# YukunXia/SuperPoint-Stereo-Visual-Odometry

Measured on AMD Instinct MI355X. Metric: stereo frames/sec (1241x376 KITTI), higher is better.
Workload: dtype f32

## Files before the change

### superpoint-stereo-visual-odometry_amd/csrc/conv_wino4.hip.h

```cpp
#pragma once
#include <hip/hip_runtime.h>
#include <stdint.h>
#include <type_traits>
#include <vector>
#include "conv_mfma.hip.h"

#ifndef WINO4_LEAD
#define WINO4_LEAD 6
#endif
#ifndef WINO4_PRIO
#define WINO4_PRIO 1
#endif
#ifndef WINO4_H1_STEPS
#define WINO4_H1_STEPS 6
#endif
#ifndef WINO4_H1_START
#define WINO4_H1_START 3
#endif
#ifndef WINO4_H1_STRIDE
#define WINO4_H1_STRIDE 5
#endif
#ifndef WINO4_H2_START
#define WINO4_H2_START 4
#endif
#ifndef WINO4_H2_STRIDE
#define WINO4_H2_STRIDE 8
#endif
#ifndef WINO4_ABL
#define WINO4_ABL 0
#endif

#ifndef SPVO_STATIC_BANDS
#define SPVO_STATIC_BANDS 1
#endif

namespace spvo {

template <int TB>
struct Wino4TileT {
  static constexpr int CK = 4, TH = 8 * TB, TW = 32, LW = TW + 8, LH = TH + 2, NT = 16 * TB, NTH = 256 * TB;
  static constexpr int IN_FLOATS = CK * LH * LW;
  static constexpr int U_FLOATS = 36 * CK * CO_TILE;
  static constexpr int V_FLOATS = 10 * TB * 64 * 4;
  static constexpr int RAW_OFF = 0, U_OFF = 2 * IN_FLOATS, V_OFF = U_OFF + 2 * U_FLOATS;
  static constexpr int LDS_BYTES = (V_OFF + 2 * V_FLOATS) * 4 + 16;
};
using Wino4Tile = Wino4TileT<2>;

inline std::vector<float> pack_conv_weights_wino4(const float *w, const float *bias, int cout, int cin) {
  constexpr int CK = Wino4Tile::CK;
  const int co_tiles = (cout + CO_TILE - 1) / CO_TILE, nch = cin / CK;
  std::vector<float> out((size_t)co_tiles * nch * Wino4Tile::U_FLOATS + (size_t)co_tiles * CO_TILE, 0.f);
  static const double G[6][3] = {{0.25, 0, 0}, {-1.0 / 6, -1.0 / 6, -1.0 / 6}, {-1.0 / 6, 1.0 / 6, -1.0 / 6},
                                 {1.0 / 24, 1.0 / 12, 1.0 / 6}, {1.0 / 24, -1.0 / 12, 1.0 / 6}, {0, 0, 1}};
  for (int ct = 0; ct < co_tiles; ++ct)
    for (int o = 0; o < CO_TILE; ++o) {
      const int co = ct * CO_TILE + o;
      if (co >= cout) continue;
      out[(size_t)co_tiles * nch * Wino4Tile::U_FLOATS + co] = bias[co];
// ... 11 lines not shown
          }
      }
    }
  return out;
}

__device__ __forceinline__ void wino4_in6(const float x0, const float x1, const float x2, const float x3, const float x4, const float x5, float (&o)[6]) {
  const float e = fmaf(-4.f, x2, x4), od = fmaf(-4.f, x1, x3), e2 = x4 - x2, o2 = x3 - x1;
  o[0] = fmaf(4.f, x0, fmaf(-5.f, x2, x4));
  o[1] = e + od;
  o[2] = e - od;
  o[3] = fmaf(2.f, o2, e2);
  o[4] = fmaf(-2.f, o2, e2);
  o[5] = fmaf(4.f, x1, fmaf(-5.f, x3, x5));
}
__device__ __forceinline__ void wino4_out4(const float m0, const float m1, const float m2, const float m3, const float m4, const float m5, float (&y)[4]) {
  const float a = m1 + m2, b = m1 - m2, c = m3 + m4, d = m3 - m4;
  y[0] = (m0 + a) + c;
  y[1] = fmaf(2.f, d, b);
  y[2] = fmaf(4.f, c, a);
  y[3] = fmaf(8.f, d, b) + m5;
}

typedef float wino4_f32x2 __attribute__((ext_vector_type(2)));
__device__ __forceinline__ void wino4_out4(const wino4_f32x2 m0, const wino4_f32x2 m1, const wino4_f32x2 m2, const wino4_f32x2 m3, const wino4_f32x2 m4,
                                           const wino4_f32x2 m5, wino4_f32x2 (&y)[4]) {
  const wino4_f32x2 a = m1 + m2, b = m1 - m2, c = m3 + m4, d = m3 - m4;
  y[0] = (m0 + a) + c;
  y[1] = __builtin_elementwise_fma(wino4_f32x2{2.f, 2.f}, d, b);
  y[2] = __builtin_elementwise_fma(wino4_f32x2{4.f, 4.f}, c, a);
  y[3] = __builtin_elementwise_fma(wino4_f32x2{8.f, 8.f}, d, b) + m5;
}

template <bool POOL, bool RELU, int TAG = 0, int TB = 2>
__global__ __launch_bounds__(256 * TB, TB) void conv_wino4_kernel(const ConvArgs a) {
  using T = Wino4TileT<TB>;
  constexpr int CK = T::CK, LW = T::LW, LH = T::LH, LW4 = LW / 4, NTH = T::NTH;
  constexpr int IN_V4 = T::IN_FLOATS / 4;
  constexpr int U_V4 = T::U_FLOATS / 4;
  constexpr int NIT_U = (U_V4 + NTH - 1) / NTH;
  typedef float f32x2 __attribute__((ext_vector_type(2)));
  typedef float f32x4v __attribute__((ext_vector_type(4)));

  extern __shared__ __attribute__((aligned(16))) float smem[];

  const int tid = threadIdx.x;
  const int lane = tid & 63;
  const int c16 = lane & 15, g4 = lane >> 4;
  const int wave = __builtin_amdgcn_readfirstlane(tid >> 6);
  const int cq = wave & 3, tb = wave >> 2;
  const size_t in_plane = (size_t)a.in_hp * a.in_wp;
  const size_t out_plane = (size_t)a.out_hp * a.out_wp;
  const int n_tiles = a.tiles_x * a.tiles_y * a.co_tiles * a.batch;

  struct TileRef { const float *in_base, *w_base; int x0, y0, ct, img; };
  auto decode = [&](int id) {
    TileRef t;
    const int tx = id % a.tiles_x;
    id /= a.tiles_x;
    const int ty = id % a.tiles_y;
    id /= a.tiles_y;
    t.ct = id % a.co_tiles;
    t.img = id / a.co_tiles;
    t.x0 = tx * T::TW;
    t.y0 = ty * T::TH;
    t.in_base = a.in + ((size_t)t.img * a.in_ctot + a.in_coff) * in_plane + (size_t)(t.y0 + PADY - 1) * a.in_wp + (t.x0 + PADX - 4);
    t.w_base = a.wpack + (size_t)t.ct * a.n_chunks * T::U_FLOATS;
    return t;
  };

  auto raw_piece_off = [&](int idx) {
    idx = min(idx, IN_V4 - 1);
    const int ci = idx / (LH * LW4);
    const int rem = idx - ci * (LH * LW4);
    const int r = rem / LW4;
    const int q = rem - r * LW4;
    return 4u * (unsigned)(ci * (int)in_plane + r * a.in_wp + q * 4);
  };
  constexpr int R0 = NTH - 256;
  const unsigned roff0 = raw_piece_off(tid), roff1 = raw_piece_off(NTH + (tid - R0));
  const bool raw2 = tid >= R0 && NTH + (tid - R0) < IN_V4;
  auto issue_raw = [&](const TileRef &t, int chunk, float *buf) {
    const char *inb = reinterpret_cast<const char *>(t.in_base + (size_t)chunk * CK * in_plane);
    glds16(reinterpret_cast<const float *>(inb + roff0), buf + (wave * 64) * 4);
    if (raw2) glds16(reinterpret_cast<const float *>(inb + roff1), buf + (NTH + (wave - R0 / 64) * 64) * 4);
  };
  const unsigned uoff = 16u * (unsigned)tid;
  auto issue_u = [&](const TileRef &t, int chunk, float *buf) {
    const char *wb = reinterpret_cast<const char *>(t.w_base + (size_t)chunk * T::U_FLOATS);
#pragma unroll
    for (int it = 0; it < NIT_U; ++it)
      if (it < NIT_U - 1 || tid < U_V4 - (NIT_U - 1) * NTH) glds16(reinterpret_cast<const float *>(wb + (uoff + 16u * NTH * it)), buf + (it * NTH + wave * 64) * 4);
  };

  const int x_ci = TB == 2 ? (wave & 3) : 2 * (wave & 1) + ((lane >> 4) & 1), x_tile = TB == 2 ? (lane & 31) : (lane & 15), x_h = lane >> 5;
  const int x_trow = x_tile >> 3, x_tcol = x_tile & 7;
  const int raw_off = x_ci * (LH * LW) + (4 * x_trow + 3 * x_h) * LW + 4 * x_tcol + 3;
  const int v_off = x_h * (1280 * TB) + (x_tile >> 4) * 256 + (16 * x_ci + (x_tile & 15)) * 4;
  float xr[3][6];
  f32x4v xa[3];
  float xs0[3], xs1[3];
  auto xf_step = [&](const float *raw, float *vb, int st) {
    if (st < 3) {
      const float *d = raw + raw_off + st * LW;
      xs0[st] = d[0];
      xa[st] = *reinterpret_cast<const f32x4v *>(d + 1);
      xs1[st] = d[5];
    } else if (st < 6) {
      const int r = st - 3;
      wino4_in6(xs0[r], xa[r][0], xa[r][1], xa[r][2], xa[r][3], xs1[r], xr[r]);
    } else if (st == 6) {
#pragma unroll
      for (int r = 0; r < 3; ++r)
#pragma unroll
        for (int c = 0; c < 3; ++c) {
          typedef unsigned u32x2s __attribute__((ext_vector_type(2)));
          const u32x2s sw = __builtin_amdgcn_permlane32_swap(__float_as_uint(xr[r][c]), __float_as_uint(xr[r][c + 3]), false, false);
          xr[r][c] = __uint_as_float(sw[0]);
          xr[r][c + 3] = __uint_as_float(sw[1]);
        }
    } else {
      const int c = st - 7;
      float o[6];
      wino4_in6(xr[0][c], xr[1][c], xr[2][c], xr[0][c + 3], xr[1][c + 3], xr[2][c + 3], o);
#pragma unroll
      for (int i = 0; i < 6; ++i) vb[v_off + ((3 * i + c) >> 2) * (256 * TB) + ((3 * i + c) & 3)] = o[i];
    }
  };

  const int a_lane = cq * 64 + lane;
  const int b_lane = tb * 64 + lane;

  const int band = blockIdx.x & 7;
  auto wgs_before = [&](int b) { return min(b, (int)gridDim.x & 7) + b * ((int)gridDim.x >> 3); };
// ... 49 lines not shown
  Cursor cr = cu;
  advance(cr);
  asm volatile("s_waitcnt vmcnt(0)\n\ts_barrier" ::: "memory");
  if (wave < 2 * TB) {
#pragma unroll
    for (int st = 0; st < 10; ++st) xf_step(smem + T::RAW_OFF, smem + T::V_OFF, st);
  } else {
#pragma unroll
    for (int st = 0; st < WINO4_H1_STEPS; ++st) xf_step(smem + T::RAW_OFF + T::IN_FLOATS, smem + T::V_OFF + T::V_FLOATS, st);
  }
  asm volatile("s_waitcnt lgkmcnt(0)\n\ts_barrier" ::: "memory");
  if (cr.id < n_tiles) issue_raw(cr.t, cr.chunk, smem + T::RAW_OFF);
  advance(cr);

#ifdef WINO_STAMPS
  unsigned long long st_dma = 0, st_bar = 0, st_mfma = 0, st_epi = 0, st_items = 0, st_post = 0, st_bar_xf = 0, st_mfma_xf = 0;
  const unsigned long long st_t0 = __builtin_amdgcn_s_memtime(), st_r0 = __builtin_amdgcn_s_memrealtime();
  int st_c = 0;
#endif
  int k = 0;
  bool drained = false;
  constexpr unsigned OOB = 0xFFFFFFFFu;

  while (tile_id < n_tiles) {
    if (a.sched) {
      if (tid == 0) dyn_fetch = band_lo(band) + band_wgs(band) + atomicAdd(a.sched + band, 1);
    } else {
      nxt_id = tile_id + gridDim.x;
    }

    f32x4v acc[36];
    auto item = [&](auto first_tag, bool publish) {
      constexpr bool FIRST = decltype(first_tag)::value;
      const bool XF = __builtin_amdgcn_readfirstlane((wave >> TB) == (k & 1) ? 1 : 0) != 0;
#ifdef WINO_STAMPS
      const unsigned long long ts0 = __builtin_amdgcn_s_memtime();
#endif
      if (!drained) asm volatile("s_waitcnt vmcnt(0)" ::: "memory");
      drained = false;
#ifdef WINO_STAMPS
      const unsigned long long ts1 = __builtin_amdgcn_s_memtime();
#endif
      if (publish && tid == 0) *sched_slot = dyn_fetch < band_hi(band) ? dyn_fetch : n_tiles;
      asm volatile("s_waitcnt lgkmcnt(0)\n\ts_barrier" ::: "memory");
      if (publish) nxt_id = __builtin_amdgcn_readfirstlane(*sched_slot);
#ifdef WINO_STAMPS
      const unsigned long long ts2 = __builtin_amdgcn_s_memtime();
      st_dma += ts1 - ts0; st_bar += ts2 - ts1;
      if (st_c == 1) st_post += ts1 - ts0;
      if (XF) st_bar_xf += ts2 - ts1;
#endif
      const float *ub = smem + T::U_OFF + (k & 1) * T::U_FLOATS;
      const float *vb = smem + T::V_OFF + (k & 1) * T::V_FLOATS;
      float *u_next = smem + T::U_OFF + ((k + 1) & 1) * T::U_FLOATS;
      const float *raw_next2 = smem + T::RAW_OFF + (k & 1) * T::IN_FLOATS;
      float *raw_next3 = smem + T::RAW_OFF + ((k + 1) & 1) * T::IN_FLOATS;
      float *v_next = smem + T::V_OFF + ((k + 1) & 1) * T::V_FLOATS;
      const f32x4v *ub4 = reinterpret_cast<const f32x4v *>(ub) + a_lane;
      const f32x4v *vb4 = reinterpret_cast<const f32x4v *>(vb) + b_lane;
      constexpr int LEAD = WINO4_LEAD;
      f32x4v av[9], bv[10];
      auto b_piece = [](int p) { return 5 * (p / 18) + ((p % 18) >> 2); };
#pragma unroll
      for (int p = 0; p < ((WINO4_ABL & 8) ? 36 : LEAD); ++p) {
        if ((WINO4_ABL & 8) && k > 0) break;
        if ((p & 3) == 0) av[p >> 2] = ub4[(p >> 2) * 256];
        if (p == 0 || b_piece(p) != b_piece(p - 1)) bv[b_piece(p)] = vb4[b_piece(p) * (64 * TB)];
      }
#pragma unroll
      for (int p = 0; p < 36; ++p) {
        const int ph = p / 18, pq = p % 18, pos = 6 * (pq / 3) + 3 * ph + pq % 3;
        const float a_op = av[p >> 2][p & 3], b_op = bv[b_piece(p)][pq & 3];
#if WINO4_PRIO
#if WINO4_PRIO == 1
        if (p == 0) asm volatile("s_setprio 3");
        if (p == 9) asm volatile("s_setprio 2");
        if (p == 18) asm volatile("s_setprio 1");
        if (p == 27) asm volatile("s_setprio 0");
#elif WINO4_PRIO == 2
        if (p == 0) asm volatile("s_setprio 3");
        if (tb == 0) { if (p == 6) asm volatile("s_setprio 2"); if (p == 15) asm volatile("s_setprio 1"); if (p == 24) asm volatile("s_setprio 0"); }
        else { if (p == 12) asm volatile("s_setprio 2"); if (p == 24) asm volatile("s_setprio 1"); }
#elif WINO4_PRIO == 3
        if (p == 0) asm volatile("s_setprio 1");
        if (p == 18) asm volatile("s_setprio 0");
#elif WINO4_PRIO == 4
        if (tb == 0) { if (p == 0) asm volatile("s_setprio 2"); if (p == 12) asm volatile("s_setprio 1"); if (p == 24) asm volatile("s_setprio 0"); }
        else { if (p == 0) asm volatile("s_setprio 3"); if (p == 12) asm volatile("s_setprio 2"); if (p == 24) asm volatile("s_setprio 1"); }
#endif
#endif
        if (FIRST) acc[pos] = __builtin_amdgcn_mfma_f32_16x16x4f32(a_op, b_op, f32x4v{0.f, 0.f, 0.f, 0.f}, 0, 0, 0);
        else acc[pos] = __builtin_amdgcn_mfma_f32_16x16x4f32(a_op, b_op, acc[pos], 0, 0, 0);
        __builtin_amdgcn_sched_barrier(0);
        if (!(WINO4_ABL & 2) && p == 1 && cu.id < n_tiles) issue_u(cu.t, cu.chunk, u_next);
        if (!(WINO4_ABL & 4) && p == 4 && cr.id < n_tiles) issue_raw(cr.t, cr.chunk, raw_next3);
        const int q = p + LEAD;
        if (!(WINO4_ABL & 8) && q < 36) {
          if ((q & 3) == 0) av[q >> 2] = ub4[(q >> 2) * 256];
          if (b_piece(q) != b_piece(q - 1)) bv[b_piece(q)] = vb4[b_piece(q) * (64 * TB)];
        }
        if (!(WINO4_ABL & 1) && XF && p >= WINO4_H1_START && p < WINO4_H1_START + WINO4_H1_STEPS * WINO4_H1_STRIDE && (p - WINO4_H1_START) % WINO4_H1_STRIDE == 0)
          xf_step(raw_next2, v_next, (p - WINO4_H1_START) / WINO4_H1_STRIDE);
        if (!(WINO4_ABL & 1) && !XF && p >= WINO4_H2_START && p < WINO4_H2_START + (10 - WINO4_H1_STEPS) * WINO4_H2_STRIDE && (p - WINO4_H2_START) % WINO4_H2_STRIDE == 0)
          xf_step(raw_next2, v_next, WINO4_H1_STEPS + (p - WINO4_H2_START) / WINO4_H2_STRIDE);
        __builtin_amdgcn_sched_barrier(0);
      }
      advance(cu);
      advance(cr);
      ++k;
#ifdef WINO_STAMPS
      { const unsigned long long dt = __builtin_amdgcn_s_memtime() - ts2; st_mfma += dt; if (XF) st_mfma_xf += dt; }
      ++st_items; ++st_c;
#endif
    };
#ifdef WINO_STAMPS
    st_c = 0;
#endif
    item(std::true_type{}, false);
    for (int c = 1; c < a.n_chunks; ++c) item(std::false_type{}, a.sched != nullptr && c == 1);

#ifdef WINO_STAMPS
    const unsigned long long te0 = __builtin_amdgcn_s_memtime();
#endif
    asm volatile("s_waitcnt vmcnt(0)" ::: "memory");
    drained = true;

    const int co0 = cur.ct * CO_TILE + cq * 16 + 4 * g4;
    float *co_base = a.out + (((size_t)cur.img * a.out_ctot + a.out_coff) + (size_t)cur.ct * CO_TILE + cq * 16) * out_plane;
    const __amdgpu_buffer_rsrc_t rsrc = __builtin_amdgcn_make_buffer_rsrc(co_base, 0, 0x7FFFFFFF, 0x00020000);
    const int oplane = (int)out_plane;
    const int kmax = a.cout - co0;
    const float *bias_p = a.wpack + (size_t)a.co_tiles * a.n_chunks * T::U_FLOATS + min(co0, a.cout - 1);
    const int trow = 2 * tb + (c16 >> 3), tcol = c16 & 7;
    auto relu = [](float v) { return RELU ? __builtin_amdgcn_fmed3f(v, 0.f, __builtin_inff()) : v; };
    const int oy = cur.y0 + 4 * trow, ox = cur.x0 + 4 * tcol;
#pragma unroll
    for (int rp = 0; rp < 2; ++rp) {
      typedef wino4_f32x2 f32x2;
// ... 70 lines not shown
```

### superpoint-stereo-visual-odometry_amd/csrc/spvo_core.hip

```cpp
#include "spvo_internal.hip.h"
#include <mutex>
#include "conv_mfma.hip.h"
#include "conv_f16.hip.h"
#include "conv_bf16x3.hip.h"
#include "conv_wino2.hip.h"
#include "conv_wino4.hip.h"
#include "heads.hip.h"
#include "conv_i8.hip.h"
#include "conv_i8_fused.hip.h"
#include "heads_i8.hip.h"

namespace spvo_int {

thread_local std::string g_error;
HostDiag g_diag;

int fail(spvo_ctx *c, int code, const char *fmt, ...) {
  char buf[512];
  va_list ap;
  va_start(ap, fmt);
  vsnprintf(buf, sizeof buf, fmt, ap);
  va_end(ap);
  if (c) c->error = buf;
  g_error = buf;
  return code;
}

int stage_id(spvo_ctx *c, const std::string &name) {
  for (size_t i = 0; i < c->stages.size(); ++i)
    if (c->stages[i].name == name) return (int)i;
  Stage s;
  s.name = name;
  c->stages.push_back(s);
  return (int)c->stages.size() - 1;
}

namespace {
const char *const kTuningNames[] = {"winograd", "wino4", "wino_narrow", "wino_dynamic", "winograd_min_tiles", "wino4_min_tiles", "merge_siblings", "heads_fused",
                                    "heads_on_net", "heads_split", "match_fused", "fp32_split", "prematch", "spin_wait", "trunk_timing", "solve_timing", "nms_first", "upload_side", "inject_launch_failure", "int8_fused", "pair_always", "preprocess_fused", "heads_keep_raw", "tail_streams", "solve_collect_first", "graphs", "solve_fuse", "solve_keep", "sift_describe_form", "sift_pair_waves_per_cu"};
constexpr int kTuningCount = sizeof kTuningNames / sizeof kTuningNames[0];
std::mutex g_tuning_mutex;
bool g_tuning_set[kTuningCount] = {};
int g_tuning_value[kTuningCount] = {};
int tuning_index(const char *name) {
  for (int i = 0; name && i < kTuningCount; ++i)
    if (std::strcmp(name, kTuningNames[i]) == 0) return i;
  return -1;
}
}
int tuning(const char *name, int dflt) {
  const int i = tuning_index(name);
  if (i < 0) return dflt;
  std::lock_guard<std::mutex> lock(g_tuning_mutex);
  return g_tuning_set[i] ? g_tuning_value[i] : dflt;
}

bool spin_wait_enabled() { return tuning("spin_wait", 0) != 0; }
hipError_t wait_event(hipEvent_t ev) {
  if (spin_wait_enabled()) {
    for (long spins = 0; spins < 20000000; ++spins) {
      const hipError_t e = hipEventQuery(ev);
      if (e != hipErrorNotReady) return e;
      __builtin_ia32_pause();
    }
  }
  return hipEventSynchronize(ev);
}

hipEvent_t get_event(spvo_ctx *c) {
  if (!c->free_events.empty()) {
    hipEvent_t e = c->free_events.back();
// ... 715 lines not shown
        op.co_tiles = (op.cout + CO_TILE - 1) / CO_TILE;
        int ck_unused;
        choose_variant(op.ks, ti.H, ti.W, op.co_tiles, c->cfg.max_batch, pool, c->num_cus, &op.wr, &op.wc, &ck_unused, true);
        const std::vector<unsigned short> pk = pack_conv_weights_s3(w, b, op.cout, op.cin, op.ks, ckg);
        int rc = dev_alloc(c, &op.d_ws3, pk.size(), false);
        if (rc) return rc;
        HIP_TRY(c, hipMemcpy(op.d_ws3, pk.data(), pk.size() * sizeof(unsigned short), hipMemcpyHostToDevice));
        continue;
      }
      if (op.cin == 1) {
        if (pool || add) return fail(c, SPVO_ERR_IO, "op %u: single-channel-input layers have no pooling / residual form", i);
        int rc = dev_alloc(c, &op.d_w, (size_t)op.cout * taps, false);
        if (rc) return rc;
        if ((rc = dev_alloc(c, &op.d_b, op.cout, false))) return rc;
        HIP_TRY(c, hipMemcpy(op.d_w, w, (size_t)op.cout * taps * 4, hipMemcpyHostToDevice));
        HIP_TRY(c, hipMemcpy(op.d_b, b, (size_t)op.cout * 4, hipMemcpyHostToDevice));
        continue;
      }
      op.co_tiles = (op.cout + CO_TILE - 1) / CO_TILE;
      choose_variant(op.ks, ti.H, ti.W, op.co_tiles, c->cfg.max_batch, pool, c->num_cus, &op.wr, &op.wc, &op.ck);
      {
        const bool wino_on = tuning("winograd", 1) != 0;
        const long wtiles = (long)((ti.W + WinoTile::TW - 1) / WinoTile::TW) * ((ti.H + WinoTile::TH - 1) / WinoTile::TH) * op.co_tiles * c->cfg.max_batch;
        const long min_tiles = tuning("winograd_min_tiles", 3 * c->num_cus / 4);
        const bool eligible = wino_on && op.ks == 3 && !bn && !add && (op.cin % WinoTile::CK) == 0 && (!pool || ((ti.H % 2) == 0 && (ti.W % 2) == 0));
        op.wino = eligible && wtiles >= min_tiles;
        if (eligible && !op.wino && tuning("wino_narrow", 1) && (op.cout % 32) == 0 && 3 * wtiles >= min_tiles) op.wino = op.wino_narrow = true;
      }
      const bool dynamic_tiles = tuning("wino_dynamic", 1) != 0;
      if (op.wino && !op.wino_narrow && (op.cin % Wino4Tile::CK) == 0 && (((ti.H | ti.W) & 1) == 0 || !pool) && tuning("wino4", 1)) {
        const long t4 = (long)((ti.W + Wino4Tile::TW - 1) / Wino4Tile::TW) * ((ti.H + Wino4Tile::TH - 1) / Wino4Tile::TH) * op.co_tiles * c->cfg.max_batch;
        if (t4 >= tuning("wino4_min_tiles", 3 * c->num_cus / 4)) {
          op.wino4 = true;
          op.ck = Wino4Tile::CK;
          op.n_chunks = op.cin / Wino4Tile::CK;
          const std::vector<float> pk = pack_conv_weights_wino4(w, b, op.cout, op.cin);
          int rc = dev_alloc(c, &op.d_w, pk.size(), false);
          if (rc) return rc;
          HIP_TRY(c, hipMemcpy(op.d_w, pk.data(), pk.size() * 4, hipMemcpyHostToDevice));
          if (dynamic_tiles && (rc = dev_alloc(c, &op.d_sched, 16))) return rc;
          continue;
        }
      }
      if (op.wino) {
        op.ck = WinoTile::CK;
        op.n_chunks = op.cin / op.ck;
        if (op.wino_narrow) op.co_tiles = op.cout / 32;
        const std::vector<float> pk = pack_conv_weights_wino2(w, b, op.cout, op.cin, op.wino_narrow ? 32 : CO_TILE);
        int rc = dev_alloc(c, &op.d_w, pk.size(), false);
        if (rc) return rc;
        HIP_TRY(c, hipMemcpy(op.d_w, pk.data(), pk.size() * 4, hipMemcpyHostToDevice));
        if (dynamic_tiles && (rc = dev_alloc(c, &op.d_sched, 16))) return rc;
        continue;
      }
      if (op.cin % op.ck) return fail(c, SPVO_ERR_IO, "op %u: cin %d is not a multiple of %d", i, op.cin, op.ck);
      op.n_chunks = op.cin / op.ck;
      const std::vector<float> pk = pack_conv_weights(w, b, op.cout, op.cin, op.ks, op.ck);
      std::vector<float> bp((size_t)op.co_tiles * CO_TILE, 0.f);
      for (int o = 0; o < op.cout; ++o) bp[o] = b[o];
      int rc = dev_alloc(c, &op.d_w, pk.size(), false);
      if (rc) return rc;
      if ((rc = dev_alloc(c, &op.d_b, bp.size(), false))) return rc;
      HIP_TRY(c, hipMemcpy(op.d_w, pk.data(), pk.size() * 4, hipMemcpyHostToDevice));
      HIP_TRY(c, hipMemcpy(op.d_b, bp.data(), bp.size() * 4, hipMemcpyHostToDevice));
    } else if (op.type == OP_MAXPOOL) {
      std::snprintf(name, sizeof name, "pool:%u", i);
// ... 185 lines not shown
```

### superpoint-stereo-visual-odometry_amd/csrc/spvo_internal.hip.h

```cpp
#pragma once
#include <hip/hip_runtime.h>

#include <algorithm>
#include <cmath>
#include <cstdarg>
#include <cstdio>
#include <cstdlib>
#include <cstring>
#include <string>
#include <vector>
#include <deque>
#include <time.h>

#include "../../include/spvo.h"
#include "spvo_types.hip.h"

#pragma GCC visibility push(hidden)
namespace spvo { struct BriskLongPair; struct BriskShortPair; }
using namespace spvo;

#include "launch_segments.hip.h"

namespace spvo_int {

constexpr int RING = 8;
constexpr int MAX_INFLIGHT = 6;
constexpr int N_SLOTS = 16;
constexpr int N_BIN_SLOTS = 10;
constexpr int N_SIFT_SLOTS = 10;
constexpr int SIFT_SLOT_MAX = 32768;
constexpr int BIN_COUNTER_INTS = 16;
constexpr int HAM_KEY_SHIFT = 22;

struct Tensor {
  int ch = 0, level = 0, H = 0, W = 0, hp = 0, wp = 0;
  bool nhwc = false;
  bool f16 = false;
  bool i8 = false;
  bool s3 = false;
  float scale = 0.f;
  float *d = nullptr;
  float *dr[RING] = {};
  size_t per_image = 0;
};

enum { OP_CONV = 1, OP_MAXPOOL = 2, OP_L2NORM = 3, OP_DWCONV = 4 };
enum { FLAG_RELU = 1, FLAG_POOL = 2, FLAG_BN = 4, FLAG_ADD = 8 };

struct Op {
  int type = 0, in = 0, out = 0, out_c_off = 0, in_c_off = 0, cin = 0, cout = 0, ks = 0, flags = 0;
  int ck = 0, n_chunks = 0, co_tiles = 0, wr = 0, wc = 0;
  int residual = 0;
  bool merged = false;
  bool wino = false;
  bool wino_narrow = false;
  bool wino4 = false;
  bool dominant = false;
  float *d_w = nullptr, *d_b = nullptr, *d_bn_scale = nullptr, *d_bn_shift = nullptr;
  int *d_sched = nullptr;
  _Float16 *d_w16 = nullptr;
  int8_t *d_w8 = nullptr;
  unsigned short *d_ws3 = nullptr;
  int *d_wq32 = nullptr;
  int *d_wsel = nullptr;
  int fused_dw = -1;
  bool fused_stem = false;
  bool fused_away = false;
  float *d_qm = nullptr;
  float inv_s_out = 0.f, s_res = 0.f;
  double flops_per_image = 0;
  int stage = -1;
};

struct Stage {
  std::string name;
  double total_ms = 0;
  long long calls = 0;
  double flops = 0, bytes = 0;
  double flops_sum = 0, bytes_sum = 0;
};

struct Pending { int stage; hipEvent_t e0, e1; double flops = 0, bytes = 0; };

struct SlotState {
  int n = 0;
  bool filled = false;
  int *d_n = nullptr;
  unsigned long long gen = 0;
};
// ... 551 lines not shown
```

### superpoint-stereo-visual-odometry_amd/csrc/spvo_net_f32.hip

```cpp
#include "spvo_internal.hip.h"
#include "conv_mfma.hip.h"
#include "conv_wino2.hip.h"
#include "conv_wino4.hip.h"
#include "heads.hip.h"

namespace spvo_int {

template <int KS, int CK, int WR, int WC, bool POOL, bool RELU, int EPI = 0, int MINW = 1, int TAG = 0>
int launch_conv_instance(spvo_ctx *c, ConvArgs args, hipStream_t stream) {
  using T = ConvTile<KS, CK, WR, WC>;
  auto k = conv_mfma_kernel<KS, CK, WR, WC, POOL, RELU, MINW, 0, EPI, TAG>;
  static int per_cu[64] = {};
  const int dev = c->cfg.device & 63;
  if (!per_cu[dev]) {
    HIP_TRY(c, hipFuncSetAttribute((const void *)k, hipFuncAttributeMaxDynamicSharedMemorySize, T::LDS_BYTES));
    int n = 0;
    HIP_TRY(c, hipOccupancyMaxActiveBlocksPerMultiprocessor(&n, (const void *)k, 256, T::LDS_BYTES));
    per_cu[dev] = std::max(n, 1);
  }
  const int n_tiles = args.tiles_x * args.tiles_y * args.co_tiles * args.batch;
  const int grid = std::min(n_tiles, c->num_cus * per_cu[dev]);
  hipLaunchKernelGGL(k, dim3(grid), dim3(256), T::LDS_BYTES, stream, args);
  HIP_TRY(c, hipGetLastError());
  return SPVO_OK;
// ... 26 lines not shown

template <bool POOL, bool RELU, int TAG, bool ODD = false, bool NARROW = false>
int launch_conv_wino_instance(spvo_ctx *c, const ConvArgs &args, hipStream_t stream) {
  static bool ready[64] = {};
  const int dev = c->cfg.device & 63;
  const int n_tiles = args.tiles_x * args.tiles_y * args.co_tiles * args.batch;
  const int rounds = (n_tiles + c->num_cus - 1) / c->num_cus;
  const int grid = (n_tiles + rounds - 1) / rounds;
  auto k = conv_wino2_kernel<POOL, RELU, TAG, ODD, NARROW>;
  if (!ready[dev]) {
    HIP_TRY(c, hipFuncSetAttribute((const void *)k, hipFuncAttributeMaxDynamicSharedMemorySize, WINO2_LDS_BYTES));
    ready[dev] = true;
  }
  ConvArgs a2 = args;
  if (rounds < 2 || args.n_chunks < 4) a2.sched = nullptr;
  hipLaunchKernelGGL(k, dim3(grid), dim3(512), WINO2_LDS_BYTES, stream, a2);
  HIP_TRY(c, hipGetLastError());
  return SPVO_OK;
}

int launch_conv_wino_sel(spvo_ctx *c, const ConvArgs &args, bool relu, bool pool, bool dominant, bool narrow, hipStream_t stream) {
  const ConvArgs &a = args;
  if (narrow) {
    if (!pool && ((a.H | a.W) & 1)) return relu ? launch_conv_wino_instance<false, true, 0, true, true>(c, args, stream) : launch_conv_wino_instance<false, false, 0, true, true>(c, args, stream);
    if (pool) return relu ? launch_conv_wino_instance<true, true, 0, false, true>(c, args, stream) : launch_conv_wino_instance<true, false, 0, false, true>(c, args, stream);
    return relu ? launch_conv_wino_instance<false, true, 0, false, true>(c, args, stream) : launch_conv_wino_instance<false, false, 0, false, true>(c, args, stream);
  }
  if (!pool && ((a.H | a.W) & 1)) return relu ? launch_conv_wino_instance<false, true, 0, true>(c, args, stream) : launch_conv_wino_instance<false, false, 0, true>(c, args, stream);
  if (dominant && relu) return pool ? launch_conv_wino_instance<true, true, 1, false>(c, args, stream) : launch_conv_wino_instance<false, true, 1, false>(c, args, stream);
  if (pool) return relu ? launch_conv_wino_instance<true, true, 0, false>(c, args, stream) : launch_conv_wino_instance<true, false, 0, false>(c, args, stream);
  return relu ? launch_conv_wino_instance<false, true, 0, false>(c, args, stream) : launch_conv_wino_instance<false, false, 0, false>(c, args, stream);
}

template <bool POOL, bool RELU, int TAG>
int launch_conv_wino4_instance(spvo_ctx *c, const ConvArgs &args, hipStream_t stream) {
  static bool ready[64] = {};
  const int dev = c->cfg.device & 63;
  auto k = conv_wino4_kernel<POOL, RELU, TAG>;
  if (!ready[dev]) {
    HIP_TRY(c, hipFuncSetAttribute((const void *)k, hipFuncAttributeMaxDynamicSharedMemorySize, Wino4Tile::LDS_BYTES));
    ready[dev] = true;
  }
  const int n_tiles = args.tiles_x * args.tiles_y * args.co_tiles * args.batch;
  const int rounds = (n_tiles + c->num_cus - 1) / c->num_cus;
  const int grid = (n_tiles + rounds - 1) / rounds;
  ConvArgs a2 = args;
  if (rounds < 2 || args.n_chunks < 5) a2.sched = nullptr;
  hipLaunchKernelGGL(k, dim3(grid), dim3(512), Wino4Tile::LDS_BYTES, stream, a2);
  HIP_TRY(c, hipGetLastError());
  return SPVO_OK;
}

int launch_conv_wino4(spvo_ctx *c, const ConvArgs &a, int batch, bool relu, bool pool, bool dominant, hipStream_t stream) {
  ConvArgs args = a;
  args.tiles_x = (a.W + Wino4Tile::TW - 1) / Wino4Tile::TW;
  args.tiles_y = (a.H + Wino4Tile::TH - 1) / Wino4Tile::TH;
  args.batch = batch;
  if (pool && ((a.H | a.W) & 1)) return fail(c, SPVO_ERR_INVALID, "F(4x4) kernel: pooled layer with odd size");
  if (dominant && relu) return pool ? launch_conv_wino4_instance<true, true, 1>(c, args, stream) : launch_conv_wino4_instance<false, true, 1>(c, args, stream);
  if (pool) return relu ? launch_conv_wino4_instance<true, true, 0>(c, args, stream) : launch_conv_wino4_instance<true, false, 0>(c, args, stream);
  return relu ? launch_conv_wino4_instance<false, true, 0>(c, args, stream) : launch_conv_wino4_instance<false, false, 0>(c, args, stream);
}

int launch_conv_wino(spvo_ctx *c, const ConvArgs &a, int batch, bool relu, bool pool, bool dominant, bool narrow, hipStream_t stream) {
  ConvArgs args = a;
  args.tiles_x = (a.W + WinoTile::TW - 1) / WinoTile::TW;
  args.tiles_y = (a.H + WinoTile::TH - 1) / WinoTile::TH;
  args.batch = batch;
  return launch_conv_wino_sel(c, args, relu, pool, dominant, narrow, stream);
}

int launch_conv(spvo_ctx *c, const Op &op, int img0, int batch, hipStream_t stream) {
  const Tensor &ti = c->tensors[op.in];
  const Tensor &to = c->tensors[op.out];
  const float *tin = ring_ptr(c, ti, img0);
  float *tout = ring_ptr(c, to, img0);
  const bool relu = op.flags & FLAG_RELU, pool = op.flags & FLAG_POOL;
  const int epi = (op.flags & FLAG_BN) ? 1 : (op.flags & FLAG_ADD) ? 2 : 0;
  if (op.type == OP_DWCONV) {
    dim3 grid((ti.W + 255) / 256, (ti.H + 3) / 4, batch * op.cout);
    if (relu)
      hipLaunchKernelGGL(dwconv3x3_kernel<true>, grid, dim3(256), 0, stream, tin, tout, op.d_w, op.d_b, op.cout, ti.H, ti.W, ti.hp, ti.wp);
    else
      hipLaunchKernelGGL(dwconv3x3_kernel<false>, grid, dim3(256), 0, stream, tin, tout, op.d_w, op.d_b, op.cout, ti.H, ti.W, ti.hp, ti.wp);
    HIP_TRY(c, hipGetLastError());
    return SPVO_OK;
  }
  if (op.cin == 1) {
    dim3 grid((ti.W + 63) / 64, (ti.H + 3) / 4, batch);
#define SPVO_FIRST(KS, RELU) hipLaunchKernelGGL((conv_first_kernel<KS, RELU>), grid, dim3(256), 0, stream, tin, tout, op.d_w, op.d_b, \
                                                op.d_bn_scale, op.d_bn_shift, ti.H, ti.W, ti.hp, ti.wp, to.ch, op.out_c_off, op.cout, 0)
    if (op.ks == 3 && !op.d_bn_scale) {
      dim3 g4((ti.W + 255) / 256, (ti.H + 3) / 4, batch);
      if (relu) hipLaunchKernelGGL(conv_first4_kernel<true>, g4, dim3(256), 0, stream, tin, tout, op.d_w, op.d_b, ti.H, ti.W, ti.hp, ti.wp, to.ch, op.out_c_off, op.cout);
      else hipLaunchKernelGGL(conv_first4_kernel<false>, g4, dim3(256), 0, stream, tin, tout, op.d_w, op.d_b, ti.H, ti.W, ti.hp, ti.wp, to.ch, op.out_c_off, op.cout);
    } else if (op.ks == 3) { if (relu) SPVO_FIRST(3, true); else SPVO_FIRST(3, false); }
    else            { if (relu) SPVO_FIRST(1, true); else SPVO_FIRST(1, false); }
#undef SPVO_FIRST
    HIP_TRY(c, hipGetLastError());
    return SPVO_OK;
  }
  ConvArgs a;
  a.in = tin; a.out = tout; a.wpack = op.d_w; a.bias = op.d_b;
  a.H = ti.H; a.W = ti.W;
  a.in_hp = ti.hp; a.in_wp = ti.wp; a.in_ctot = ti.ch; a.in_coff = op.in_c_off;
  a.out_hp = to.hp; a.out_wp = to.wp; a.out_ctot = to.ch; a.out_coff = op.out_c_off;
  a.cout = op.cout; a.n_chunks = op.n_chunks; a.co_tiles = op.co_tiles;
  a.tiles_x = a.tiles_y = 0;
  a.batch = batch;
  a.sched = op.d_sched;
  if (op.wino4) return launch_conv_wino4(c, a, batch, relu, pool, op.dominant, stream);
  if (op.wino) return launch_conv_wino(c, a, batch, relu, pool, op.dominant, op.wino_narrow, stream);
  const int key = op.ks * 10000 + op.ck * 100 + op.wr * 20 + op.wc * 2 + (pool ? 1 : 0);
  if (epi) {
    a.bn_scale = op.d_bn_scale; a.bn_shift = op.d_bn_shift;
    if (epi == 2) a.residual = ring_ptr(c, c->tensors[op.residual], img0);
    switch (key) {
      case 11644: return launch_conv_epi<2, 2, false>(c, a, batch, epi, stream);
      case 11624: return launch_conv_epi<1, 2, false>(c, a, batch, epi, stream);
      case 11622: return launch_conv_epi<1, 1, false>(c, a, batch, epi, stream);
      case 11645: return launch_conv_epi<2, 2, true>(c, a, batch, epi, stream);
      case 11643: return launch_conv_epi<2, 1, true>(c, a, batch, epi, stream);
      default: return fail(c, SPVO_ERR_INVALID, "no conv kernel variant for key %d with epilogue %d", key, epi);
    }
  }
  switch (key) {
    case 30844: return launch_conv_variant<3, 8, 2, 2, false, 1>(c, a, batch, relu, stream, op.dominant);
    case 30842: return launch_conv_variant<3, 8, 2, 1, false, 2>(c, a, batch, relu, stream, op.dominant);
    case 30824: return launch_conv_variant<3, 8, 1, 2, false, 2>(c, a, batch, relu, stream, op.dominant);
    case 30822: return launch_conv_variant<3, 8, 1, 1, false, 4>(c, a, batch, relu, stream, op.dominant);
    case 30845: return launch_conv_variant<3, 8, 2, 2, true, 1>(c, a, batch, relu, stream, op.dominant);
    case 30843: return launch_conv_variant<3, 8, 2, 1, true, 2>(c, a, batch, relu, stream, op.dominant);
    case 11644: return launch_conv_variant<1, 16, 2, 2, false>(c, a, batch, relu, stream);
    case 11624: return launch_conv_variant<1, 16, 1, 2, false>(c, a, batch, relu, stream);
    case 11622: return launch_conv_variant<1, 16, 1, 1, false>(c, a, batch, relu, stream);
    case 11645: return launch_conv_variant<1, 16, 2, 2, true>(c, a, batch, relu, stream);
    case 11643: return launch_conv_variant<1, 16, 2, 1, true>(c, a, batch, relu, stream);
    default: return fail(c, SPVO_ERR_INVALID, "no conv kernel variant for key %d", key);
  }
}

int launch_op(spvo_ctx *c, const Op &op, int img0, int batch, hipStream_t stream) {
  if (op.merged || op.fused_away) return SPVO_OK;
  const Tensor &ti = c->tensors[op.in];
// ... 92 lines not shown
```

Measured before the change: 1517.

## Hand-schedule Winograd F(4x4) item loop with explicit LDS reads and fine waitcnts

After: 1559 (median of 6 runs). +2.8%, better.

```diff
diff --git a/superpoint-stereo-visual-odometry_amd/csrc/conv_wino4.hip.h b/superpoint-stereo-visual-odometry_amd/csrc/conv_wino4.hip.h
--- a/superpoint-stereo-visual-odometry_amd/csrc/conv_wino4.hip.h
+++ b/superpoint-stereo-visual-odometry_amd/csrc/conv_wino4.hip.h
@@ -2,6 +2,7 @@
 #include <hip/hip_runtime.h>
 #include <stdint.h>
 #include <type_traits>
+#include <utility>
 #include <vector>
 #include "conv_mfma.hip.h"
 
@@ -25,6 +26,9 @@
 #endif
 #ifndef WINO4_H2_STRIDE
 #define WINO4_H2_STRIDE 8
+#endif
+#ifndef WINO4_ITEM_LEAD
+#define WINO4_ITEM_LEAD 6
 #endif
 #ifndef WINO4_ABL
 #define WINO4_ABL 0
@@ -102,12 +106,33 @@
   y[3] = __builtin_elementwise_fma(wino4_f32x2{8.f, 8.f}, d, b) + m5;
 }
 
-template <bool POOL, bool RELU, int TAG = 0, int TB = 2>
+constexpr int wino4_b_piece(int p) { return 5 * (p / 18) + ((p % 18) >> 2); }
+constexpr bool wino4_slot_reads_a(int q) { return (q & 3) == 0; }
+constexpr bool wino4_slot_reads_b(int q) { return q == 0 || wino4_b_piece(q) != wino4_b_piece(q - 1); }
+constexpr int wino4_reads_before(int q_end) {
+  int n = 0;
+  for (int q = 0; q < q_end && q < 36; ++q) n += (wino4_slot_reads_a(q) ? 1 : 0) + (wino4_slot_reads_b(q) ? 1 : 0);
+  return n;
+}
+constexpr int wino4_first_slot_b(int piece) { return 18 * (piece / 5) + 4 * (piece % 5); }
+constexpr int wino4_wait_count(int p, int lead) {
+  const int issued = wino4_reads_before(p + lead);
+  const int qa = p & ~3, qb = wino4_first_slot_b(wino4_b_piece(p));
+  const int ia = wino4_reads_before(qa);
+  const int ib = wino4_reads_before(qb) + (wino4_slot_reads_a(qb) ? 1 : 0);
+  const int n = issued - 1 - (ia > ib ? ia : ib);
+  return n < 0 ? 0 : (n > 15 ? 15 : n);
+}
+template <class F, int... P>
+__device__ __forceinline__ void wino4_for_each(F &&f, std::integer_sequence<int, P...>) { (f(std::integral_constant<int, P>{}), ...); }
+
+template <bool POOL, bool RELU, int TAG = 0, int TB = 2, bool ITEM = true>
 __global__ __launch_bounds__(256 * TB, TB) void conv_wino4_kernel(const ConvArgs a) {
   using T = Wino4TileT<TB>;
   constexpr int CK = T::CK, LW = T::LW, LH = T::LH, LW4 = LW / 4, NTH = T::NTH;
   constexpr int IN_V4 = T::IN_FLOATS / 4;
   constexpr int U_V4 = T::U_FLOATS / 4;
+  constexpr bool NEW_ITEM = ITEM && !(WINO4_ABL & 8);
   constexpr int NIT_U = (U_V4 + NTH - 1) / NTH;
   typedef float f32x2 __attribute__((ext_vector_type(2)));
   typedef float f32x4v __attribute__((ext_vector_type(4)));
@@ -170,6 +195,7 @@
   float xr[3][6];
   f32x4v xa[3];
   float xs0[3], xs1[3];
+  f32x2 xs2[3];
   auto xf_step = [&](const float *raw, float *vb, int st) {
     if (st < 3) {
       const float *d = raw + raw_off + st * LW;
@@ -285,7 +311,7 @@
     f32x4v acc[36];
     auto item = [&](auto first_tag, bool publish) {
       constexpr bool FIRST = decltype(first_tag)::value;
-      const bool XF = __builtin_amdgcn_readfirstlane((wave >> TB) == (k & 1) ? 1 : 0) != 0;
+      const bool XF = NEW_ITEM ? (((wave >> TB) ^ k) & 1) == 0 : __builtin_amdgcn_readfirstlane((wave >> TB) == (k & 1) ? 1 : 0) != 0;
 #ifdef WINO_STAMPS
       const unsigned long long ts0 = __builtin_amdgcn_s_memtime();
 #endif
@@ -311,52 +337,121 @@
       float *v_next = smem + T::V_OFF + ((k + 1) & 1) * T::V_FLOATS;
       const f32x4v *ub4 = reinterpret_cast<const f32x4v *>(ub) + a_lane;
       const f32x4v *vb4 = reinterpret_cast<const f32x4v *>(vb) + b_lane;
-      constexpr int LEAD = WINO4_LEAD;
-      f32x4v av[9], bv[10];
-      auto b_piece = [](int p) { return 5 * (p / 18) + ((p % 18) >> 2); };
-#pragma unroll
-      for (int p = 0; p < ((WINO4_ABL & 8) ? 36 : LEAD); ++p) {
-        if ((WINO4_ABL & 8) && k > 0) break;
-        if ((p & 3) == 0) av[p >> 2] = ub4[(p >> 2) * 256];
-        if (p == 0 || b_piece(p) != b_piece(p - 1)) bv[b_piece(p)] = vb4[b_piece(p) * (64 * TB)];
-      }
-#pragma unroll
-      for (int p = 0; p < 36; ++p) {
-        const int ph = p / 18, pq = p % 18, pos = 6 * (pq / 3) + 3 * ph + pq % 3;
-        const float a_op = av[p >> 2][p & 3], b_op = bv[b_piece(p)][pq & 3];
+      if constexpr (NEW_ITEM) {
+        constexpr int LEAD = WINO4_ITEM_LEAD;
+        static_assert(LEAD >= 1 && LEAD <= 36, "WINO4_ITEM_LEAD");
+        static_assert(WINO4_PRIO <= 1, "the other priority schedules exist in the ITEM = 0 form only");
+        f32x4v av[9], bv[10];
+        f32x2 bh[2];
+        static_assert(WINO4_H1_STEPS >= 6, "the row reads and the row pass that waits for them run in one item");
+        const int xf_s = ((wave >> TB) ^ k ^ 1) & 1;
+        auto is_xf = [xf_s]() __attribute__((always_inline)) { int t = xf_s; asm volatile("" : "+s"(t)); return t != 0; };
+        const unsigned ra = (unsigned)(uintptr_t)(const __attribute__((address_space(3))) void *)(raw_next2 + raw_off);
+        const unsigned ua = (unsigned)(uintptr_t)(const __attribute__((address_space(3))) void *)ub4;
+        const unsigned va = (unsigned)(uintptr_t)(const __attribute__((address_space(3))) void *)vb4;
+        auto read_slot = [&av, &bv, &bh, ua, va](auto qc) __attribute__((always_inline)) {
+          constexpr int q = decltype(qc)::value;
+          if constexpr (q < 36 && wino4_slot_reads_a(q)) asm volatile("ds_read_b128 %0, %1 offset:%2" : "=v"(av[q >> 2]) : "v"(ua), "n"((q >> 2) * 256 * 16));
+          constexpr int j = wino4_b_piece(q < 36 ? q : 35);
+          if constexpr (q < 36 && wino4_slot_reads_b(q) && j % 5 == 4) asm volatile("ds_read_b64 %0, %1 offset:%2" : "=v"(bh[j / 5]) : "v"(va), "n"(j * 64 * TB * 16));
+          if constexpr (q < 36 && wino4_slot_reads_b(q) && j % 5 != 4) asm volatile("ds_read_b128 %0, %1 offset:%2" : "=v"(bv[j]) : "v"(va), "n"(j * 64 * TB * 16));
+        };
+        auto step = [&](auto pc) __attribute__((always_inline)) {
+          constexpr int p = decltype(pc)::value;
+          constexpr int ph = p / 18, pq = p % 18, pos = 6 * (pq / 3) + 3 * ph + pq % 3, bj = wino4_b_piece(p);
+          constexpr bool half = bj % 5 == 4;
+          if constexpr (wino4_slot_reads_a(p) || wino4_slot_reads_b(p)) {
+            if constexpr (half) asm volatile("s_waitcnt lgkmcnt(%2)" : "+v"(av[p >> 2]), "+v"(bh[bj / 5]) : "n"(wino4_wait_count(p, LEAD)));
+            else asm volatile("s_waitcnt lgkmcnt(%2)" : "+v"(av[p >> 2]), "+v"(bv[bj]) : "n"(wino4_wait_count(p, LEAD)));
+          }
+          const float a_op = av[p >> 2][p & 3];
+          float b_op;
+          if constexpr (half) b_op = bh[bj / 5][pq & 3];
+          else b_op = bv[bj][pq & 3];
+#if WINO4_PRIO
+          if constexpr (p == 0) asm volatile("s_setprio 3");
+          if constexpr (p == 9) asm volatile("s_setprio 2");
+          if constexpr (p == 18) asm volatile("s_setprio 1");
+          if constexpr (p == 27) asm volatile("s_setprio 0");
+#endif
+          if (FIRST) acc[pos] = __builtin_amdgcn_mfma_f32_16x16x4f32(a_op, b_op, f32x4v{0.f, 0.f, 0.f, 0.f}, 0, 0, 0);
+          else acc[pos] = __builtin_amdgcn_mfma_f32_16x16x4f32(a_op, b_op, acc[pos], 0, 0, 0);
+          __builtin_amdgcn_sched_barrier(0);
+          if (!(WINO4_ABL & 2) && p == 1 && cu.id < n_tiles) issue_u(cu.t, cu.chunk, u_next);
+          if (!(WINO4_ABL & 4) && p == 4 && cr.id < n_tiles) issue_raw(cr.t, cr.chunk, raw_next3);
+          read_slot(std::integral_constant<int, p + LEAD>{});
+          if constexpr (!(WINO4_ABL & 1) && p >= WINO4_H1_START && p < WINO4_H1_START + WINO4_H1_STEPS * WINO4_H1_STRIDE && (p - WINO4_H1_START) % WINO4_H1_STRIDE == 0) {
+            constexpr int st = (p - WINO4_H1_START) / WINO4_H1_STRIDE;
+            if (is_xf()) {
+              if constexpr (st < 3) {
+                asm volatile("ds_read2_b32 %0, %1 offset0:%2 offset1:%3" : "=v"(xs2[st]) : "v"(ra), "n"(st * LW), "n"(st * LW + 5));
+                asm volatile("ds_read_b128 %0, %1 offset:%2" : "=v"(xa[st]) : "v"(ra), "n"((st * LW + 1) * 4));
+              } else {
+                if constexpr (st < 6) {
+                  constexpr int p_rd = p - 3 * WINO4_H1_STRIDE;
+                  constexpr int n = wino4_reads_before(p + LEAD + 1) - wino4_reads_before(p_rd + LEAD + 1) + 2 * (5 - st);
+                  asm volatile("s_waitcnt lgkmcnt(%2)" : "+v"(xs2[st - 3]), "+v"(xa[st - 3]) : "n"(n > 15 ? 15 : n));
+                  xs0[st - 3] = xs2[st - 3][0];
+                  xs1[st - 3] = xs2[st - 3][1];
+                }
+                xf_step(raw_next2, v_next, st);
+              }
+            }
+          }
+          if constexpr (!(WINO4_ABL & 1) && p >= WINO4_H2_START && p < WINO4_H2_START + (10 - WINO4_H1_STEPS) * WINO4_H2_STRIDE && (p - WINO4_H2_START) % WINO4_H2_STRIDE == 0)
+            if (!is_xf()) xf_step(raw_next2, v_next, WINO4_H1_STEPS + (p - WINO4_H2_START) / WINO4_H2_STRIDE);
+          __builtin_amdgcn_sched_barrier(0);
+        };
+        wino4_for_each(read_slot, std::make_integer_sequence<int, LEAD>{});
+        wino4_for_each(step, std::make_integer_sequence<int, 36>{});
+      } else {
+        constexpr int LEAD = WINO4_LEAD;
+        f32x4v av[9], bv[10];
+        auto b_piece = [](int p) { return 5 * (p / 18) + ((p % 18) >> 2); };
+#pragma unroll
+        for (int p = 0; p < ((WINO4_ABL & 8) ? 36 : LEAD); ++p) {
+          if ((WINO4_ABL & 8) && k > 0) break;
+          if ((p & 3) == 0) av[p >> 2] = ub4[(p >> 2) * 256];
+          if (p == 0 || b_piece(p) != b_piece(p - 1)) bv[b_piece(p)] = vb4[b_piece(p) * (64 * TB)];
+        }
+#pragma unroll
+        for (int p = 0; p < 36; ++p) {
+          const int ph = p / 18, pq = p % 18, pos = 6 * (pq / 3) + 3 * ph + pq % 3;
+          const float a_op = av[p >> 2][p & 3], b_op = bv[b_piece(p)][pq & 3];
 #if WINO4_PRIO
 #if WINO4_PRIO == 1
-        if (p == 0) asm volatile("s_setprio 3");
-        if (p == 9) asm volatile("s_setprio 2");
-        if (p == 18) asm volatile("s_setprio 1");
-        if (p == 27) asm volatile("s_setprio 0");
+          if (p == 0) asm volatile("s_setprio 3");
+          if (p == 9) asm volatile("s_setprio 2");
+          if (p == 18) asm volatile("s_setprio 1");
+          if (p == 27) asm volatile("s_setprio 0");
 #elif WINO4_PRIO == 2
-        if (p == 0) asm volatile("s_setprio 3");
-        if (tb == 0) { if (p == 6) asm volatile("s_setprio 2"); if (p == 15) asm volatile("s_setprio 1"); if (p == 24) asm volatile("s_setprio 0"); }
-        else { if (p == 12) asm volatile("s_setprio 2"); if (p == 24) asm volatile("s_setprio 1"); }
+          if (p == 0) asm volatile("s_setprio 3");
+          if (tb == 0) { if (p == 6) asm volatile("s_setprio 2"); if (p == 15) asm volatile("s_setprio 1"); if (p == 24) asm volatile("s_setprio 0"); }
+          else { if (p == 12) asm volatile("s_setprio 2"); if (p == 24) asm volatile("s_setprio 1"); }
 #elif WINO4_PRIO == 3
-        if (p == 0) asm volatile("s_setprio 1");
-        if (p == 18) asm volatile("s_setprio 0");
+          if (p == 0) asm volatile("s_setprio 1");
+          if (p == 18) asm volatile("s_setprio 0");
 #elif WINO4_PRIO == 4
-        if (tb == 0) { if (p == 0) asm volatile("s_setprio 2"); if (p == 12) asm volatile("s_setprio 1"); if (p == 24) asm volatile("s_setprio 0"); }
-        else { if (p == 0) asm volatile("s_setprio 3"); if (p == 12) asm volatile("s_setprio 2"); if (p == 24) asm volatile("s_setprio 1"); }
-#endif
-#endif
-        if (FIRST) acc[pos] = __builtin_amdgcn_mfma_f32_16x16x4f32(a_op, b_op, f32x4v{0.f, 0.f, 0.f, 0.f}, 0, 0, 0);
-        else acc[pos] = __builtin_amdgcn_mfma_f32_16x16x4f32(a_op, b_op, acc[pos], 0, 0, 0);
-        __builtin_amdgcn_sched_barrier(0);
-        if (!(WINO4_ABL & 2) && p == 1 && cu.id < n_tiles) issue_u(cu.t, cu.chunk, u_next);
-        if (!(WINO4_ABL & 4) && p == 4 && cr.id < n_tiles) issue_raw(cr.t, cr.chunk, raw_next3);
-        const int q = p + LEAD;
-        if (!(WINO4_ABL & 8) && q < 36) {
-          if ((q & 3) == 0) av[q >> 2] = ub4[(q >> 2) * 256];
-          if (b_piece(q) != b_piece(q - 1)) bv[b_piece(q)] = vb4[b_piece(q) * (64 * TB)];
+          if (tb == 0) { if (p == 0) asm volatile("s_setprio 2"); if (p == 12) asm volatile("s_setprio 1"); if (p == 24) asm volatile("s_setprio 0"); }
+          else { if (p == 0) asm volatile("s_setprio 3"); if (p == 12) asm volatile("s_setprio 2"); if (p == 24) asm volatile("s_setprio 1"); }
+#endif
+#endif
+          if (FIRST) acc[pos] = __builtin_amdgcn_mfma_f32_16x16x4f32(a_op, b_op, f32x4v{0.f, 0.f, 0.f, 0.f}, 0, 0, 0);
+          else acc[pos] = __builtin_amdgcn_mfma_f32_16x16x4f32(a_op, b_op, acc[pos], 0, 0, 0);
+          __builtin_amdgcn_sched_barrier(0);
+          if (!(WINO4_ABL & 2) && p == 1 && cu.id < n_tiles) issue_u(cu.t, cu.chunk, u_next);
+          if (!(WINO4_ABL & 4) && p == 4 && cr.id < n_tiles) issue_raw(cr.t, cr.chunk, raw_next3);
+          const int q = p + LEAD;
+          if (!(WINO4_ABL & 8) && q < 36) {
+            if ((q & 3) == 0) av[q >> 2] = ub4[(q >> 2) * 256];
+            if (b_piece(q) != b_piece(q - 1)) bv[b_piece(q)] = vb4[b_piece(q) * (64 * TB)];
+          }
+          if (!(WINO4_ABL & 1) && XF && p >= WINO4_H1_START && p < WINO4_H1_START + WINO4_H1_STEPS * WINO4_H1_STRIDE && (p - WINO4_H1_START) % WINO4_H1_STRIDE == 0)
+            xf_step(raw_next2, v_next, (p - WINO4_H1_START) / WINO4_H1_STRIDE);
+          if (!(WINO4_ABL & 1) && !XF && p >= WINO4_H2_START && p < WINO4_H2_START + (10 - WINO4_H1_STEPS) * WINO4_H2_STRIDE && (p - WINO4_H2_START) % WINO4_H2_STRIDE == 0)
+            xf_step(raw_next2, v_next, WINO4_H1_STEPS + (p - WINO4_H2_START) / WINO4_H2_STRIDE);
+          __builtin_amdgcn_sched_barrier(0);
         }
-        if (!(WINO4_ABL & 1) && XF && p >= WINO4_H1_START && p < WINO4_H1_START + WINO4_H1_STEPS * WINO4_H1_STRIDE && (p - WINO4_H1_START) % WINO4_H1_STRIDE == 0)
-          xf_step(raw_next2, v_next, (p - WINO4_H1_START) / WINO4_H1_STRIDE);
-        if (!(WINO4_ABL & 1) && !XF && p >= WINO4_H2_START && p < WINO4_H2_START + (10 - WINO4_H1_STEPS) * WINO4_H2_STRIDE && (p - WINO4_H2_START) % WINO4_H2_STRIDE == 0)
-          xf_step(raw_next2, v_next, WINO4_H1_STEPS + (p - WINO4_H2_START) / WINO4_H2_STRIDE);
-        __builtin_amdgcn_sched_barrier(0);
       }
       advance(cu);
       advance(cr);
diff --git a/superpoint-stereo-visual-odometry_amd/csrc/spvo_core.hip b/superpoint-stereo-visual-odometry_amd/csrc/spvo_core.hip
--- a/superpoint-stereo-visual-odometry_amd/csrc/spvo_core.hip
+++ b/superpoint-stereo-visual-odometry_amd/csrc/spvo_core.hip
@@ -36,7 +36,7 @@
 }
 
 namespace {
-const char *const kTuningNames[] = {"winograd", "wino4", "wino_narrow", "wino_dynamic", "winograd_min_tiles", "wino4_min_tiles", "merge_siblings", "heads_fused",
+const char *const kTuningNames[] = {"winograd", "wino4", "wino4_item", "wino_narrow", "wino_dynamic", "winograd_min_tiles", "wino4_min_tiles", "merge_siblings", "heads_fused",
                                     "heads_on_net", "heads_split", "match_fused", "fp32_split", "prematch", "spin_wait", "trunk_timing", "solve_timing", "nms_first", "upload_side", "inject_launch_failure", "int8_fused", "pair_always", "preprocess_fused", "heads_keep_raw", "tail_streams", "solve_collect_first", "graphs", "solve_fuse", "solve_keep", "sift_describe_form", "sift_pair_waves_per_cu"};
 constexpr int kTuningCount = sizeof kTuningNames / sizeof kTuningNames[0];
 std::mutex g_tuning_mutex;
@@ -818,6 +818,7 @@
         const long t4 = (long)((ti.W + Wino4Tile::TW - 1) / Wino4Tile::TW) * ((ti.H + Wino4Tile::TH - 1) / Wino4Tile::TH) * op.co_tiles * c->cfg.max_batch;
         if (t4 >= tuning("wino4_min_tiles", 3 * c->num_cus / 4)) {
           op.wino4 = true;
+          op.wino4_item = tuning("wino4_item", 1) != 0;
           op.ck = Wino4Tile::CK;
           op.n_chunks = op.cin / Wino4Tile::CK;
           const std::vector<float> pk = pack_conv_weights_wino4(w, b, op.cout, op.cin);
diff --git a/superpoint-stereo-visual-odometry_amd/csrc/spvo_internal.hip.h b/superpoint-stereo-visual-odometry_amd/csrc/spvo_internal.hip.h
--- a/superpoint-stereo-visual-odometry_amd/csrc/spvo_internal.hip.h
+++ b/superpoint-stereo-visual-odometry_amd/csrc/spvo_internal.hip.h
@@ -55,6 +55,7 @@
   bool wino = false;
   bool wino_narrow = false;
   bool wino4 = false;
+  bool wino4_item = true;
   bool dominant = false;
   float *d_w = nullptr, *d_b = nullptr, *d_bn_scale = nullptr, *d_bn_shift = nullptr;
   int *d_sched = nullptr;
diff --git a/superpoint-stereo-visual-odometry_amd/csrc/spvo_net_f32.hip b/superpoint-stereo-visual-odometry_amd/csrc/spvo_net_f32.hip
--- a/superpoint-stereo-visual-odometry_amd/csrc/spvo_net_f32.hip
+++ b/superpoint-stereo-visual-odometry_amd/csrc/spvo_net_f32.hip
@@ -82,11 +82,11 @@
   return relu ? launch_conv_wino_instance<false, true, 0, false>(c, args, stream) : launch_conv_wino_instance<false, false, 0, false>(c, args, stream);
 }
 
-template <bool POOL, bool RELU, int TAG>
+template <bool POOL, bool RELU, int TAG, bool ITEM>
 int launch_conv_wino4_instance(spvo_ctx *c, const ConvArgs &args, hipStream_t stream) {
   static bool ready[64] = {};
   const int dev = c->cfg.device & 63;
-  auto k = conv_wino4_kernel<POOL, RELU, TAG>;
+  auto k = conv_wino4_kernel<POOL, RELU, TAG, 2, ITEM>;
   if (!ready[dev]) {
     HIP_TRY(c, hipFuncSetAttribute((const void *)k, hipFuncAttributeMaxDynamicSharedMemorySize, Wino4Tile::LDS_BYTES));
     ready[dev] = true;
@@ -101,15 +101,20 @@
   return SPVO_OK;
 }
 
-int launch_conv_wino4(spvo_ctx *c, const ConvArgs &a, int batch, bool relu, bool pool, bool dominant, hipStream_t stream) {
+template <bool ITEM>
+int launch_conv_wino4_sel(spvo_ctx *c, const ConvArgs &args, bool relu, bool pool, bool dominant, hipStream_t stream) {
+  if (dominant && relu) return pool ? launch_conv_wino4_instance<true, true, 1, ITEM>(c, args, stream) : launch_conv_wino4_instance<false, true, 1, ITEM>(c, args, stream);
+  if (pool) return relu ? launch_conv_wino4_instance<true, true, 0, ITEM>(c, args, stream) : launch_conv_wino4_instance<true, false, 0, ITEM>(c, args, stream);
+  return relu ? launch_conv_wino4_instance<false, true, 0, ITEM>(c, args, stream) : launch_conv_wino4_instance<false, false, 0, ITEM>(c, args, stream);
+}
+
+int launch_conv_wino4(spvo_ctx *c, const ConvArgs &a, int batch, bool relu, bool pool, bool dominant, bool new_item, hipStream_t stream) {
   ConvArgs args = a;
   args.tiles_x = (a.W + Wino4Tile::TW - 1) / Wino4Tile::TW;
   args.tiles_y = (a.H + Wino4Tile::TH - 1) / Wino4Tile::TH;
   args.batch = batch;
   if (pool && ((a.H | a.W) & 1)) return fail(c, SPVO_ERR_INVALID, "F(4x4) kernel: pooled layer with odd size");
-  if (dominant && relu) return pool ? launch_conv_wino4_instance<true, true, 1>(c, args, stream) : launch_conv_wino4_instance<false, true, 1>(c, args, stream);
-  if (pool) return relu ? launch_conv_wino4_instance<true, true, 0>(c, args, stream) : launch_conv_wino4_instance<true, false, 0>(c, args, stream);
-  return relu ? launch_conv_wino4_instance<false, true, 0>(c, args, stream) : launch_conv_wino4_instance<false, false, 0>(c, args, stream);
+  return new_item ? launch_conv_wino4_sel<true>(c, args, relu, pool, dominant, stream) : launch_conv_wino4_sel<false>(c, args, relu, pool, dominant, stream);
 }
 
 int launch_conv_wino(spvo_ctx *c, const ConvArgs &a, int batch, bool relu, bool pool, bool dominant, bool narrow, hipStream_t stream) {
@@ -159,7 +164,7 @@
   a.tiles_x = a.tiles_y = 0;
   a.batch = batch;
   a.sched = op.d_sched;
-  if (op.wino4) return launch_conv_wino4(c, a, batch, relu, pool, op.dominant, stream);
+  if (op.wino4) return launch_conv_wino4(c, a, batch, relu, pool, op.dominant, op.wino4_item, stream);
   if (op.wino) return launch_conv_wino(c, a, batch, relu, pool, op.dominant, op.wino_narrow, stream);
   const int key = op.ks * 10000 + op.ck * 100 + op.wr * 20 + op.wc * 2 + (pool ? 1 : 0);
   if (epi) {
```
